# modelscope/KAN-TTS

Measured on AMD Instinct MI355X. Metric: mel-frames/sec (SAM-BERT train), higher is better.
Workload: dtype bf16; 1 GPU; SAM-BERT full (sambert_16k.yaml zhcn) fwd+bwd+clip+Adam, batch 32/GPU, T_in 64, 14797 valid mel frames on rank 0, dropout on; global_batch=32, parallelism=dp1, launch=graph, collective_world_size=1

## Files before the change

include/kantts_hip.h:

```cpp
#ifndef KANTTS_HIP_H
#define KANTTS_HIP_H

#include <stddef.h>
#include <stdint.h>

#ifdef __cplusplus
extern "C" {
#endif

#define KANTTS_OK 0
#define KANTTS_E_BADARG (-1)
#define KANTTS_E_UNSUPPORTED (-2)
#define KANTTS_E_WORKSPACE (-3)

int kantts_abi_version(void);
const char* kantts_target_arch(void);

#define KANTTS_GEMM_MAX_SEG 4
typedef struct kantts_gemm_seg {
  const float* a;
  const float* a_gate;
  const float* b;
  int64_t a_is, a_ks;
  int64_t b_js, b_ks;
// ... 152 lines not shown
                    int64_t* lens, int B, int N, int Tp, void* stream);
int kantts_lr_gather_fwd(const float* x, const int32_t* idx, const int64_t* valid_lens, float* out, int B, int N,
                         int Tp, int C, int ldo, int out_col_offset, void* stream);
int kantts_lr_gather_bwd(const float* dout, const int32_t* cs, const int64_t* valid_lens, float* dx, int B, int N,
                         int Tp, int C, int ldo, int out_col_offset, int accumulate, void* stream);

int kantts_lr_memory_fwd(const float* aug, const float* spk, const float* emo, const int32_t* idx,
                         const int64_t* valid_lens, const float* pos_enc, float* memory, float* lr_text, float* lr_spk,
                         float* lr_emo, int B, int N, int Tp, int r, int d_t, int d_s, int d_e, void* stream);
int kantts_lr_memory_bwd(const float* d_memory, long long ldm, const int32_t* cs, const int64_t* valid_lens, float* d_aug,
                         float* d_spk, float* d_emo, int B, int N, int Tp, int r, int d_t, int d_s, int d_e, void* stream);

int kantts_fsmn_dwconv_fwd(const float* x, const float* w, const float* res, const int64_t* lens, float* y, int B,
                           int T, int C, int K, int left_pad, void* stream);
int kantts_fsmn_dwconv_fwd_rows(const float* x, const float* w, const float* res, const int64_t* lens, float* y, int B,
                                int T, int C, int K, int left_pad, int t0, int t1, void* stream);
int kantts_fsmn_dwconv_fwd_slots(const float* x, const float* w, const float* res, const int64_t* lens, float* y, int B,
                                 int T, int C, int K, int left_pad, const int32_t* t0, const int32_t* t1, int max_rows,
                                 void* stream);
int kantts_fsmn_dwconv_bwd(const float* dy, const float* x, const float* w, const int64_t* lens, float* dx,
                           float* dw_accum, float* workspace, long long ws_floats, int B, int T, int C, int K,
                           int left_pad, void* stream);
long long kantts_fsmn_dwconv_bwd_ws(int B, int T, int C, int K);
int kantts_fsmn_memory_drop_fwd(const float* c, const float* w, const float* res, const int64_t* lens, float* y, int B,
                                int T, int C, int K, int left_pad, float p1, uint64_t seed1, float p2, uint64_t seed2,
                                const uint64_t* seed_dev, void* stream);
int kantts_fsmn_memory_drop_bwd(const float* dy, const float* w, const int64_t* lens, float* dx, float* dym, int B, int T,
                                int C, int K, int left_pad, float p1, uint64_t seed1, float p2, uint64_t seed2,
                                const uint64_t* seed_dev, void* stream);
typedef struct kantts_fsmn_drop_args {
  const float* x;
  const float* w;
  const float* res;
  float* y;
  float* dym;
  float p1, p2;
  uint64_t seed1, seed2;
} kantts_fsmn_drop_args;
int kantts_fsmn_memory_drop_fwd_pair(const kantts_fsmn_drop_args* a, const kantts_fsmn_drop_args* b, const int64_t* lens,
                                     int B, int T, int C, int K, int left_pad, const uint64_t* seed_dev, void* stream);
int kantts_fsmn_memory_drop_bwd_pair(const kantts_fsmn_drop_args* a, const kantts_fsmn_drop_args* b, const int64_t* lens,
                                     int B, int T, int C, int K, int left_pad, const uint64_t* seed_dev, void* stream);

int kantts_masked_l1(const float* pred, const float* target, const int64_t* lens, float* loss_accum, float* grad,
                     int B, int T, int C, void* stream);

// ... 803 lines not shown
```

kan-tts_amd/csrc/seq.hip:

```cpp
#include "common.h"

struct EmbedArgs {
  const float* tab[4];
  int ntab;
  const int64_t* ids;
  const float* pos;
  float* out;
  float* scaled;
  int rows, T, D;
  float scale;
};

__global__ void embed_sum_kernel(const EmbedArgs a) {
  long long idx = (long long)blockIdx.x * blockDim.x + threadIdx.x;
  long long total = (long long)a.rows * a.D;
  if (idx >= total) return;
  int row = (int)(idx / a.D), d = (int)(idx % a.D);
  float s = 0.f;
  for (int k = 0; k < a.ntab; ++k) s += a.tab[k][(long long)a.ids[(long long)row * a.ntab + k] * a.D + d];
  s *= a.scale;
  if (a.scaled) a.scaled[idx] = s;
  if (a.pos) s += a.pos[(long long)(row % a.T) * a.D + d];
  a.out[idx] = s;
}
// ... 448 lines not shown
      const int t = t0 + o;
      const bool ok = t < (ROWS ? min(len, r1) : len);
      const float v = xb[(long long)(ok ? t : 0) * C + c];
      ctr[o] = ok ? v : 0.f;
    }
#pragma unroll
    for (int o = 0; o < FS_TT; ++o) {
      const int t = t0 + o;
      float acc = ctr[o];
#pragma unroll
      for (int k = 0; k < FS_K; ++k) acc = fmaf(wk[k], xin[o + k], acc);
      if (t < tlim) {
        const long long oidx = ((long long)b * T + t) * C + c;
        float outv = (t < len) ? acc : 0.f;
        if (!FLIP && res) outv += res[oidx];
        y[oidx] = outv;
      }
    }
  }
}

#define FS_CH 128
#define FS_SUB (FS_CH / 4)
__global__ __launch_bounds__(256) void fsmn_dw41_partial_kernel(const float* __restrict__ dy, const float* __restrict__ x,
                                                            const int64_t* __restrict__ lens,
                                                            float* __restrict__ part, int B, int T, int C, int lp) {
  __shared__ float sm[4][FS_K][65];
  const int b = blockIdx.y, chunk = blockIdx.x, nchunk = gridDim.x;
  const int wave = threadIdx.x >> 6, lane = threadIdx.x & 63;
  const int c0 = blockIdx.z * 64, c = c0 + lane;
  const bool cok = c < C;
  const int cc = cok ? c : 0;
  const int len = lens ? (int)min((long long)lens[b], (long long)T) : T;
  const float* xb = x + (long long)b * T * C;
  const float* db = dy + (long long)b * T * C;
  const int tbeg = chunk * FS_CH + wave * FS_SUB, tend = min(tbeg + FS_SUB, T);
  float acc[FS_K];
#pragma unroll
  for (int k = 0; k < FS_K; ++k) acc[k] = 0.f;
  for (int t0 = tbeg; t0 < tend && t0 < len; t0 += FS_TT) {
    float xin[FS_TT + FS_K - 1], dv[FS_TT];
#pragma unroll
    for (int n = 0; n < FS_TT + FS_K - 1; ++n) {
      const int ts = t0 + n - lp;
      const bool ok = cok && (ts >= 0) && (ts < len);
      const float v = xb[(long long)(ok ? ts : 0) * C + cc];
      xin[n] = ok ? v : 0.f;
    }
#pragma unroll
    for (int o = 0; o < FS_TT; ++o) {
      const int t = t0 + o;
      const bool ok = cok && (t < tend) && (t < len);
      const float v = db[(long long)(ok ? t : 0) * C + cc];
      dv[o] = ok ? v : 0.f;
    }
    __builtin_amdgcn_sched_barrier(0);
#pragma unroll
    for (int o = 0; o < FS_TT; ++o)
#pragma unroll
      for (int k = 0; k < FS_K; ++k) acc[k] = fmaf(dv[o], xin[o + k], acc[k]);
  }
#pragma unroll
  for (int k = 0; k < FS_K; ++k) sm[wave][k][lane] = acc[k];
  __syncthreads();
  float* p = part + (((long long)b * nchunk + chunk) * C + c0) * FS_K;
  const int nout = min(64, C - c0) * FS_K;
  for (int o = threadIdx.x; o < nout; o += 256) {
    const int cl = o / FS_K, k = o - cl * FS_K;
    p[o] = (sm[0][k][cl] + sm[1][k][cl]) + (sm[2][k][cl] + sm[3][k][cl]);
  }
}

#define FS_RS 8
__global__ __launch_bounds__(64 * FS_RS) void fsmn_dw_reduce_kernel(const float* __restrict__ part, float* __restrict__ dw,
                                                                    int nblk, int n) {
  __shared__ float sm[FS_RS][64];
  const int lane = threadIdx.x & 63, slice = threadIdx.x >> 6;
  const int i = blockIdx.x * 64 + lane;
  const bool ok = i < n;
  const long long ii = ok ? i : 0;
  float s0 = 0.f, s1 = 0.f, s2 = 0.f, s3 = 0.f;
  int p = slice;
  for (; p + 3 * FS_RS < nblk; p += 4 * FS_RS) {
    const float a0 = part[(long long)p * n + ii], a1 = part[(long long)(p + FS_RS) * n + ii];
    const float a2 = part[(long long)(p + 2 * FS_RS) * n + ii], a3 = part[(long long)(p + 3 * FS_RS) * n + ii];
    s0 += a0, s1 += a1, s2 += a2, s3 += a3;
  }
  for (; p < nblk; p += FS_RS) s0 += part[(long long)p * n + ii];
  sm[slice][lane] = (s0 + s1) + (s2 + s3);
  __syncthreads();
  if (slice == 0 && ok) {
    float s = 0.f;
#pragma unroll
    for (int q = 0; q < FS_RS; ++q) s += sm[q][lane];
    dw[i] += s;
  }
}

static int fs_xcd_order() {
  static const bool off = getenv("KANTTS_FIR_NO_XCD_ORDER") != nullptr;
  return off ? 0 : 1;
}

extern "C" long long kantts_fsmn_dwconv_bwd_ws(int B, int T, int C, int K) {
  if (K != FS_K) return 0;
  return (long long)B * kantts_cdiv(T, FS_CH) * C * K;
}

extern "C" int kantts_fsmn_dwconv_fwd(const float* x, const float* w, const float* res, const int64_t* lens, float* y,
                                      int B, int T, int C, int K, int left_pad, void* stream) {
  if (!x || !w || !y || B < 0 || T < 0 || C < 1 || K < 1) return KANTTS_E_BADARG;
  if (B == 0 || T == 0) return KANTTS_OK;
  const int threads = C >= 256 ? 256 : (C >= 128 ? 128 : 64);
  if (K == FS_K) {
    hipLaunchKernelGGL((fsmn_fir41_kernel<false, 0>), dim3(kantts_cdiv(T, FS_TT), B), dim3(threads), 0,
                       (hipStream_t)stream, x, w, res, lens, y, B, T, C, left_pad, fs_xcd_order(), 0, T,
                       (const int32_t*)nullptr, (const int32_t*)nullptr, 0);
  } else {
    hipLaunchKernelGGL(fsmn_dwconv_fwd_kernel<0>, dim3(kantts_cdiv(T, DW_TT), B), dim3(threads), 0, (hipStream_t)stream, x,
// ... 47 lines not shown
    const int nchunk = kantts_cdiv(T, FS_CH);
    if (dw_accum && (!workspace || ws_floats < (long long)B * nchunk * C * K)) return KANTTS_E_WORKSPACE;
    if (dx)
      hipLaunchKernelGGL((fsmn_fir41_kernel<true, 0>), dim3(kantts_cdiv(T, FS_TT), B), dim3(threads), 0, st, dy,
                         w, (const float*)nullptr, lens, dx, B, T, C, left_pad, fs_xcd_order(), 0, T, (const int32_t*)nullptr,
                         (const int32_t*)nullptr, 0);
    if (dw_accum) {
      hipLaunchKernelGGL(fsmn_dw41_partial_kernel, dim3(nchunk, B, kantts_cdiv(C, 64)), dim3(256), 0, st, dy, x, lens,
                         workspace, B, T, C, left_pad);
      hipLaunchKernelGGL(fsmn_dw_reduce_kernel, dim3(kantts_cdiv(C * K, 64)), dim3(64 * FS_RS), 0, st, workspace, dw_accum,
                         B * nchunk, C * K);
    }
  } else {
    if (dx)
      hipLaunchKernelGGL(fsmn_dwconv_bwd_dx_kernel, dim3(kantts_cdiv(T, DW_TT), B), dim3(threads), 0, st, dy, w, lens, dx,
                         B, T, C, K, left_pad);
    if (dw_accum)
      hipLaunchKernelGGL(fsmn_dwconv_bwd_dw_kernel, dim3(kantts_cdiv(T, DW_WT), B), dim3(threads), 0, st, dy, x, lens,
                         dw_accum, B, T, C, K, left_pad);
  }
  KANTTS_CHECK_LAUNCH();
}

__global__ __launch_bounds__(256) void teacher_plan_kernel(const kantts_plan_args g) {
  const long long nA = (long long)g.B * g.N, nB = (long long)g.B * g.T_mel, L = g.Tp / g.r, nC = (long long)g.B * L;
  const long long nD = (long long)g.B * g.Tp * g.depth, nE = (long long)g.B * L * g.d_mel, nF = g.B;
  const long long total = nA + nB + nC + nD + nE + nF;
  for (long long i = (long long)blockIdx.x * blockDim.x + threadIdx.x; i < total; i += (long long)gridDim.x * blockDim.x) {
    long long k = i;
    if (k < nA) {
      const int b = (int)(k / g.N), n = (int)(k % g.N);
      const long long len = min(g.in_lens[b], (long long)g.N);
      g.in_mask[k] = n >= len ? 1 : 0;
      g.prev[k] = logf((n > 0 ? (float)g.dur[k - 1] : 0.f) + 1.f);
      continue;
    }
    k -= nA;
    if (k < nB) {
      const int b = (int)(k / g.T_mel), t = (int)(k % g.T_mel);
      g.out_mask[k] = t >= min(g.out_lens[b], (long long)g.T_mel) ? 1 : 0;
      continue;
    }
    k -= nB;
    if (k < nC) {
      const int b = (int)(k / L), l = (int)(k % L);
      g.lfr_mask[k] = l >= min((g.out_lens[b] + g.r - 1) / g.r, L) ? 1 : 0;
// ... 69 lines not shown
```

kan-tts_amd/kantts/_hip/__init__.py:

```python
import ctypes
import os
from ctypes import (POINTER, Structure, c_char_p, c_float, c_int, c_int32, c_int64, c_longlong,
                    c_uint64, c_void_p)

import torch

_HERE = os.path.dirname(os.path.abspath(__file__))
LIB_PATH = os.environ.get("KANTTS_LIB") or os.path.normpath(os.path.join(_HERE, "..", "..", "libkantts_hip.so"))
_lib = None

GEMM_MAX_SEG = 4
PREC_FP32, PREC_BF16, PREC_REF = 0, 1, 2


class GemmSeg(Structure):
    _fields_ = [
        ("a", c_void_p), ("a_gate", c_void_p), ("b", c_void_p),
        ("a_is", c_int64), ("a_ks", c_int64), ("b_js", c_int64), ("b_ks", c_int64), ("b_tap", c_int64),
        ("klen", c_int32), ("ntaps", c_int32),
        ("a_tok_axis", c_int32), ("a_shift0", c_int32), ("a_shift_step", c_int32),
        ("b_tok_axis", c_int32), ("b_shift0", c_int32), ("b_shift_step", c_int32),
        ("a_drop_p", c_float), ("a_drop_seed", c_uint64),
        ("a_inner", c_int32), ("a_Tq", c_int32), ("a_Tsrc", c_int32), ("a_mul", c_int32), ("a_div", c_int32),
        ("a_up", c_int32),
# ... 329 lines not shown


class EncAttnArgs(Structure):
    _fields_ = [("x", c_void_p), ("xn", c_void_p), ("lens", c_void_p), ("rowmask", c_void_p), ("wqkv", c_void_p),
                ("bqkv", c_void_p), ("wfc", c_void_p), ("bfc", c_void_p), ("ln1_gamma", c_void_p), ("ln1_beta", c_void_p),
                ("ln1_eps", c_float), ("att_p", c_float), ("fc_p", c_float), ("att_seed", c_uint64), ("fc_seed", c_uint64),
                ("seed_dev", c_void_p), ("qkv", c_void_p), ("o", c_void_p), ("lse", c_void_p), ("y1", c_void_p),
                ("xn1", c_void_p), ("xn1_bf16", c_int32), ("mean1", c_void_p), ("rstd1", c_void_p), ("B", c_int32),
                ("L", c_int32)]


class CtcArgs(Structure):
    _fields_ = [("logits", c_void_p), ("in_lens", c_void_p), ("out_lens", c_void_p), ("ws", c_void_p), ("loss", c_void_p),
                ("grad", c_void_p), ("B", c_int32), ("T1", c_int32), ("T2", c_int32), ("blank", c_float),
                ("grad_scale", c_float)]


ROWSUM_MAX = 32


class RowSumArgs(Structure):
    _fields_ = [("n", c_int32), ("cols", c_int32), ("split", c_int32), ("rows", c_int32 * ROWSUM_MAX),
                ("src", c_void_p * ROWSUM_MAX), ("dst0", c_void_p * ROWSUM_MAX), ("dst1", c_void_p * ROWSUM_MAX)]


class FragMajorDesc(Structure):
    _fields_ = [("src_off", c_int64), ("dst_off", c_int64), ("sr", c_int64), ("sk", c_int64), ("R", c_int32),
                ("K", c_int32)]


class TapMajorDesc(Structure):
    _fields_ = [("src_off", c_int64), ("dst_off", c_int64), ("N", c_int32), ("Cin", c_int32), ("KT", c_int32),
                ("pad_", c_int32)]


def available() -> bool:
    return os.path.exists(LIB_PATH)


def lib():
    global _lib
    if _lib is None:
        if not os.path.exists(LIB_PATH):
            raise RuntimeError(
                "libkantts_hip.so is not built (%s). Run `python -c 'import __graft_entry__ as g; g.build()'` "
                "or `make -C kan-tts_amd/csrc`. There is no CPU fallback." % LIB_PATH)
# ... 12 lines not shown
        L.kantts_pnca_attn_bwd.argtypes = [p, p, i, p, p, p, p, p, p, p, p, p, p, p, i, i, i, i, i, i, f, u64, u64, p, p]
        L.kantts_attn_plan.argtypes = [i, i, i]
        L.kantts_lstm_fwd.argtypes = [p, p, p, p, p, p, p, i, i, i, i, i, i, p]
        L.kantts_attn_decode.argtypes = [p, p, p, i, i, i, p, i, p, p, i, i, i, i, i, i, i, p]
        L.kantts_lstm_cell.argtypes = [p, p, p, p, i, i, p]
        L.kantts_mas_width1.argtypes = [p, p, p, p, p, i, i, i, p]
        L.kantts_align_attn_fwd.argtypes = [p, p, p, p, p, p, i, i, i, i, p]
        L.kantts_align_attn_bwd.argtypes = [p, p, p, p, p, p, p, p, p, p, i, i, i, i, p]
        L.kantts_lstm_bwd.argtypes = [p, p, p, p, p, p, i, i, i, i, i, i, p]
        L.kantts_embed_sum_fwd.argtypes = [POINTER(c_void_p), i, p, p, p, p, i, i, i, f, p]
        L.kantts_embed_sum_bwd.argtypes = [POINTER(c_void_p), i, p, p, i, i, f, p]
        L.kantts_lr_index.argtypes = [p, p, p, p, p, p, i, i, i, p]
        L.kantts_lr_gather_fwd.argtypes = [p, p, p, p, i, i, i, i, i, i, p]
        L.kantts_lr_gather_bwd.argtypes = [p, p, p, p, i, i, i, i, i, i, i, p]
        L.kantts_lr_memory_fwd.argtypes = [p, p, p, p, p, p, p, p, p, p, i, i, i, i, i, i, i, p]
        L.kantts_lr_memory_bwd.argtypes = [p, ll, p, p, p, p, p, i, i, i, i, i, i, i, p]
        L.kantts_fsmn_dwconv_fwd.argtypes = [p, p, p, p, p, i, i, i, i, i, p]
        L.kantts_fsmn_dwconv_bwd.argtypes = [p, p, p, p, p, p, p, ll, i, i, i, i, i, p]
        L.kantts_fsmn_dwconv_bwd_ws.argtypes = [i, i, i, i]
        L.kantts_fsmn_dwconv_bwd_ws.restype = ll
        if hasattr(L, "kantts_fsmn_memory_drop_fwd") and hasattr(L, "kantts_fsmn_memory_drop_bwd"):
            L.kantts_fsmn_memory_drop_fwd.argtypes = [p, p, p, p, p, i, i, i, i, i, f, u64, f, u64, p, p]
            L.kantts_fsmn_memory_drop_bwd.argtypes = [p, p, p, p, p, i, i, i, i, i, f, u64, f, u64, p, p]
        L.kantts_masked_l1.argtypes = [p, p, p, p, p, i, i, i, p]
        L.kantts_sumsq.argtypes = [p, p, ll, p]
        L.kantts_elem_loss.argtypes = [p, p, f, i, f, p, p, ll, p]
        L.kantts_adam_step.argtypes = [p, p, p, p, ll, f, f, f, f, f, f, f, p, f, p, p]
        L.kantts_melspec_fwd.argtypes = [p, i, i, i, i, i, i, p, p, f, p, p, p, p, i, f, p, p, p]
        L.kantts_melspec_norm_fwd.argtypes = [p, i, i, i, i, i, i, p, p, f, p, p, p, p, i, f, f, f, f, i, p, p, p]
        L.kantts_melspec_bwd.argtypes = [p, p, i, i, i, i, i, i, p, p, f, p, p, p, p, i, f, p, p]
        L.kantts_melspec_norm_fwd_fm.argtypes = [p, i, i, i, i, i, i, p, p, f, p, p, p, p, i, f, f, f, f, i, i, p, p, p]
        L.kantts_melspec_bwd_fm.argtypes = [p, p, i, i, i, i, i, i, p, p, f, p, p, p, p, i, f, i, p, p]
        L.kantts_weight_norm_fwd.argtypes = [p, p, p, i, i, p]
        L.kantts_weight_norm_bwd.argtypes = [p, p, p, p, p, i, i, p]
        L.kantts_weight_norm_strided_fwd.argtypes = [p, p, p, i, i, i, ll, ll, ll, p]
        L.kantts_weight_norm_strided_bwd.argtypes = [p, p, p, p, p, i, i, i, ll, ll, ll, p]
        L.kantts_sinadd_fwd.argtypes = [p, p, ll, p]
        L.kantts_sinadd_bwd.argtypes = [p, p, p, ll, p]
        L.kantts_conv_win_launch.argtypes = [POINTER(ConvArgs), c_void_p]
        L.kantts_conv_wgrad_launch.argtypes = [POINTER(ConvWArgs), c_void_p]
        L.kantts_conv_c1_launch.argtypes = [POINTER(ConvC1Args), c_int, c_void_p]
        L.kantts_pnca_decode_step.argtypes = [p, i, p, p, p, p, p, p, i, i, i, i, i, p, i, p]
        L.kantts_step_rows.argtypes = [p, p, i, i, ll, ll, ll, ll, i, p, p]
        L.kantts_step_rowmask.argtypes = [p, p, i, i, p, p]
        L.kantts_upsample_stream.argtypes = [p, p, p, p, p, i, i, i, i, i, f, i, p]
        L.kantts_sinadd_lrelu_fwd.argtypes = [p, p, p, f, ll, p]
# ... 129 lines not shown
    "kantts_bgemm_nt", "kantts_ffn_pair", "kantts_fragmajor_bf16", "kantts_bgemm_tn", "kantts_cast_f32_bf16", "kantts_tapmajor_bf16", "kantts_relu_gate_bf16",
    "kantts_ln128_fwd", "kantts_ln128_bwd", "kantts_ln128_bwd_rows", "kantts_bgemm_nt_lnbwd", "kantts_stft_mag_bwd", "kantts_bgemm_tn_grouped", "kantts_sumsq_det",
    "kantts_pnca_decode_step", "kantts_step_rows", "kantts_step_rowmask", "kantts_upsample_stream",
    "kantts_sinadd_lrelu_fwd", "kantts_dropout2_add",
    "kantts_cconv_launch", "kantts_cconv_wgrad_launch", "kantts_cconv_wgrad_ws_floats", "kantts_act_cast_bf16",
    "kantts_ragged_rows_f32", "kantts_ragged_rows_i64", "kantts_weight_norm_tap_images",
    "kantts_weight_norm_table", "kantts_weight_norm_table_bwd", "kantts_masked_l1_many", "kantts_scale_many",
    "kantts_mean_many", "kantts_scale_to_many", "kantts_elem_loss_many", "kantts_conv_n1_launch",
    "kantts_pnca_block_fwd", "kantts_pnca_block_bwd", "kantts_pnca_block_bwd_ws_floats", "kantts_rows_sum_many",
    "kantts_melspec_tuning", "kantts_teacher_plan", "kantts_copy_roof", "kantts_pnca_attn_qkv_bwd",
    "kantts_pnca_decode_run", "kantts_pnca_decode_blob_sizes", "kantts_dur_ar_run", "kantts_dur_ar_run_f32", "kantts_ctc_attn", "kantts_ctc_attn_workspace", "kantts_enc_attn_fwd",
    "kantts_launch_tuning", "kantts_sconv_launch", "kantts_sconv_rows_launch",
    "kantts_pnca_decode_range", "kantts_lstm_fwd_range", "kantts_fsmn_dwconv_fwd_rows",
    "kantts_pnca_decode_slots", "kantts_lstm_fwd_slots", "kantts_fsmn_dwconv_fwd_slots", "kantts_scatter_rows_f32",
    "kantts_nsf_source_rows", "kantts_nsf_downs_rows", "kantts_mel_handover_rows",
    "kantts_mb_tail_rows", "kantts_sconv_sym_rows_launch", "kantts_lr_memory_fwd", "kantts_lr_memory_bwd",
    "kantts_nsf_source_end_rows", "kantts_nsf_downs_sym_rows", "kantts_nsf_draw_states", "kantts_nsf_source_wgrad",
    *FP_SYMBOLS, "kantts_fp_plan_given",
    *SPK_SYMBOLS,
    "kantts_fsmn_memory_drop_fwd", "kantts_fsmn_memory_drop_bwd",
    *PREDICTOR_PAIR_SYMBOLS,
    *CORPUS_PRIOR_SYMBOLS,
    *SYBERT_SYMBOLS,
]


_launch_tuning = [None]


def apply_launch_tuning():
    L = lib()
    env = os.environ
    want = (id(L), int(env.get("KANTTS_TN_TILE", "0") or 0), int(env.get("KANTTS_TN_SLICES", "0") or 0),
            int(env.get("KANTTS_C1_WGRAD_WGS", "0") or 0))
    if want != _launch_tuning[0]:
        rc = L.kantts_launch_tuning(want[1], max(want[2], 0), max(want[3], 0))
        if rc != 0:
            raise RuntimeError("libkantts_hip: launch_tuning failed with code %d" % rc)
        _launch_tuning[0] = want


def check(rc, what):
    if rc != 0:
        raise RuntimeError("libkantts_hip: %s failed with code %d" % (what, rc))


# ... 603 lines not shown
        _profile_families.append(("pnca_attn_qkv_bwd", e0, e1, flops, float(nbytes)))
    return ws


def rows_sum_many(problems):
    for s0 in range(0, len(problems), ROWSUM_MAX):
        chunk = problems[s0:s0 + ROWSUM_MAX]
        g = RowSumArgs()
        g.n, g.cols, g.split = len(chunk), 256, 128
        for i, (src, d0, d1) in enumerate(chunk):
            assert src.dim() == 2 and src.shape[1] == 256 and src.is_contiguous()
            g.rows[i] = int(src.shape[0])
            g.src[i], g.dst0[i], g.dst1[i] = _addr(src), _addr(d0), _addr(d1)
        check(lib().kantts_rows_sum_many(ctypes.byref(g), stream()), "rows_sum_many")


def rows_sum_accum(src, dst0, dst1):
    if deferred_tn.enabled:
        deferred_tn.rowsums.append((src, deferred_tn._desc(dst0), deferred_tn._desc(dst1)))
        return
    rows_sum_many([(src, dst0, dst1)])


TN_MAX_GROUP = 16


class _DeferredTN:

    def __init__(self):
        self.enabled = False
        self.groups = {}
        self.copies = []
        self.rowsums = []

    def add(self, key, g, a, b, c, db, seed, keep):
        self.groups.setdefault(key, []).append((g, a, b, c, db, seed, keep))

    @staticmethod
    def _desc(t):
        return (t.untyped_storage(), t.storage_offset(), tuple(t.shape), tuple(t.stride()), t.dtype, t.device)

    @staticmethod
    def _rebuild(d):
        st, off, shape, stride, dtype, dev = d
        return torch.empty(0, dtype=dtype, device=dev).set_(st, off, shape, stride)

    def shared_gradient(self, src):
        if not self.enabled:
            return src
        from .ops import gzeros

        dst = gzeros(tuple(src.shape), src.device) if src.dtype == torch.float32 else torch.empty_like(src)
        self.copies.append((self._desc(dst), self._desc(src)))
        return dst

    def flush(self):
        if not self.groups and not self.copies and not self.rowsums:
            return
        groups, self.groups = self.groups, {}
        copies, self.copies = self.copies, []
        rowsums, self.rowsums = self.rowsums, []
        self._launch([probs[s:s + TN_MAX_GROUP] for probs in groups.values() for s in range(0, len(probs), TN_MAX_GROUP)])
        if rowsums:
            rows_sum_many([(src, self._rebuild(d0), self._rebuild(d1)) for src, d0, d1 in rowsums])
        if copies:
            torch._foreach_copy_([self._rebuild(d) for d, _ in copies], [self._rebuild(s) for _, s in copies])

    def _launch(self, chunks):
        L = lib()
        for chunk in chunks:
            n = len(chunk)
            arr = lambda k: (c_void_p * n)(*[q[k] for q in chunk])
            seeds = (c_uint64 * n)(*[q[5] for q in chunk])
            g = chunk[0][0]
            g.slices = 0
            if _profile is not None:
                e0, e1 = torch.cuda.Event(enable_timing=True), torch.cuda.Event(enable_timing=True)
                e0.record()
            apply_launch_tuning()
            check(L.kantts_bgemm_tn_grouped(ctypes.byref(g), n, arr(1), arr(2), arr(3), arr(4), seeds, stream()),
                  "bgemm_tn_grouped")
            if _profile is not None:
                e1.record()
                _profile.append((e0, e1, 2.0 * g.M * g.N * g.K * g.ntaps * n))


deferred_tn = _DeferredTN()
# ... 749 lines not shown
```

kan-tts_amd/kantts/_hip/ops.py:

```python
import itertools
import os
import weakref
import math

import torch

from . import (E_UNSUPPORTED, act_cast_bf16, bgemm_nt, bgemm_tn, cconv, cconv_wgrad, check, get_precision, conv_c1, conv_n1, conv_wgrad,
               conv_win, gemm, lib, make_seg, nsf_source, nsf_source_wgrad, ptr, rng_state, stream)
from . import ops_bf16

_seed_counter = itertools.count(1)


def next_seed():
    return (torch.initial_seed() * 0x9E3779B97F4A7C15 + next(_seed_counter) * 0xD1B54A32D192ED03) & ((1 << 63) - 1)


def _c(t):
    return t if t.is_contiguous() else t.contiguous()


def distinct_stream(priority=None):
    taken = {st.cuda_stream for st in helper_streams()} | {torch.cuda.current_stream().cuda_stream}
    for _ in range(64):
# ... 100 lines not shown
                return self
            if o._stream is None:
                o._stream = _new_side_stream()
            ev = torch.cuda.Event()
            ev.record(torch.cuda.current_stream())
            o._stream.wait_event(ev)
            self.cm = torch.cuda.stream(o._stream)
            self.cm.__enter__()
            o._keep.extend(t for t in self.keep if t is not None)
            o._used = True
            return self

        def __exit__(self, *exc):
            if self.cm is not None:
                self.cm.__exit__(*exc)
            return False

    def side(self, *keep):
        return _WgradOverlap._Ctx(self, keep)

    def flush_early(self):
        from . import deferred_tn

        if not self.enabled or not (deferred_tn.groups or deferred_tn.copies or deferred_tn.rowsums):
            return
        keep = [k for probs in deferred_tn.groups.values() for q in probs for k in q[6] if k is not None]
        keep += [r[0] for r in deferred_tn.rowsums]
        with self.side(*keep):
            deferred_tn.flush()

    def join(self):
        from . import deferred_tn

        deferred_tn.flush()
        flush_weight_norm_backward()
        side_branch.join()
        side_branch.release()
        if self._used:
            ev = torch.cuda.Event()
            ev.record(self._stream)
            torch.cuda.current_stream().wait_event(ev)
            self._keep.clear()
            self._used = False


wgrad_overlap = _WgradOverlap()


_branch_streams = []

# ... 1032 lines not shown
def lr_memory_entry_points():
    return hasattr(lib(), "kantts_lr_memory_fwd")


def lr_memory(aug, spk, emo, idx, cs, valid_lens, pos_enc, r, frames=None):
    B, Tp = idx.shape
    if (LR_MEMORY["on"] and Tp % r == 0 and not pos_enc.requires_grad and lr_memory_entry_points()
            and tuple(pos_enc.shape) == (B, Tp, aug.shape[-1])
            and all(t.dtype == torch.float32 for t in (aug, spk, emo, pos_enc))):
        try:
            mem, text, fs, fe = _LRMemory.apply(_c(aug), _c(spk), _c(emo), idx, cs, valid_lens, _c(pos_enc), int(r),
                                                frames is None)
            return (mem, text) + ((fs, fe) if frames is None else tuple(frames))
        except _LRMemoryDeclined:
            pass
    text = lr_gather(aug, idx, cs, valid_lens) + pos_enc
    fs, fe = frames if frames is not None else (lr_gather(spk, idx, cs, valid_lens), lr_gather(emo, idx, cs, valid_lens))
    ds, de = spk.shape[-1], emo.shape[-1]
    mem = torch.cat([text.reshape(B, -1, r * text.shape[-1]), fs.reshape(B, -1, r * ds)[:, :, :ds],
                     fe.reshape(B, -1, r * de)[:, :, :de]], dim=-1)
    return mem, text, fs, fe


class _FsmnMemory(torch.autograd.Function):
    @staticmethod
    def forward(ctx, x, w, res, lens, lp):
        x, w = _c(x), _c(w)
        B, T, C = x.shape
        K = w.shape[-1]
        y = torch.empty_like(x)
        r = _c(res) if res is not None else None
        check(lib().kantts_fsmn_dwconv_fwd(ptr(x, torch.float32), ptr(w, torch.float32), ptr(r), ptr(lens), ptr(y), B,
                                           T, C, K, int(lp), stream()), "fsmn_dwconv_fwd")
        ctx.save_for_backward(x, w, lens)
        ctx.cfg = (B, T, C, K, int(lp), res is not None)
        return y

    @staticmethod
    def backward(ctx, dy):
        x, w, lens = ctx.saved_tensors
        B, T, C, K, lp, has_res = ctx.cfg
        dy = _c(dy)
        dx = torch.empty_like(x)
        dw = gzeros_like(w)
        ws_n = int(lib().kantts_fsmn_dwconv_bwd_ws(B, T, C, K))
        ws = torch.empty(max(ws_n, 1), device=dy.device, dtype=torch.float32)
        check(lib().kantts_fsmn_dwconv_bwd(ptr(dy, torch.float32), ptr(x), ptr(w), ptr(lens), ptr(dx), None, None, 0,
                                           B, T, C, K, lp, stream()), "fsmn_dwconv_bwd (dx)")
        with wgrad_overlap.side(dy, x, ws):
            check(lib().kantts_fsmn_dwconv_bwd(ptr(dy, torch.float32), ptr(x), ptr(w), ptr(lens), None, ptr(dw), ptr(ws),
                                               ws_n, B, T, C, K, lp, stream()), "fsmn_dwconv_bwd (dw)")
        return dx, dw, (dy if has_res else None), None, None


def fsmn_memory(x, w, lens_i64, left_pad, res=None):
    return _FsmnMemory.apply(x, w, res, lens_i64, left_pad)


class _FsmnMemoryDrop(torch.autograd.Function):

    @staticmethod
    def forward(ctx, c, w, res, lens, lp, p1, p2, res_grad=None):
        from . import rng_ptr

        c, w = _c(c), _c(w)
        B, T, C = c.shape
        K = w.shape[-1]
        r = None if res is None else _c(res)
        y = torch.empty_like(c)
        s1 = next_seed() if p1 > 0 else 0
        s2 = next_seed() if p2 > 0 else 0
        rc = lib().kantts_fsmn_memory_drop_fwd(ptr(c, torch.float32), ptr(w, torch.float32), ptr(r, torch.float32),
                                               ptr(lens), ptr(y), B, T, C, K, int(lp), float(p1), s1, float(p2), s2,
                                               rng_ptr(c.device), stream())
# ... 6 lines not shown
        check(rc, "fsmn_memory_drop_fwd")
        ctx.save_for_backward(c, w, lens)
        ctx.cfg = (B, T, C, K, int(lp), float(p1), s1, float(p2), s2, res is not None)
        ctx.res_grad = res_grad if (res is not None and res_grad is not None and res_grad.armed) else None
        return y

    @staticmethod
    def backward(ctx, dy):
        from . import rng_ptr

        c, w, lens = ctx.saved_tensors
        B, T, C, K, lp, p1, s1, p2, s2, has_res = ctx.cfg
        dy = _c(dy)
        dx, dym = torch.empty_like(c), torch.empty_like(c)
        rc = lib().kantts_fsmn_memory_drop_bwd(ptr(dy, torch.float32), ptr(w), ptr(lens), ptr(dx), ptr(dym), B, T, C, K, lp,
                                               p1, s1, p2, s2, rng_ptr(dy.device), stream())
        if rc == E_UNSUPPORTED:
            check(lib().kantts_dropout2_add(ptr(dy), None, ptr(dym), dy.numel(), p1, s1, p2, s2, rng_ptr(dy.device),
                                            stream()), "dropout2_add")
            rc = lib().kantts_fsmn_dwconv_bwd(ptr(dym), ptr(c), ptr(w), ptr(lens), ptr(dx), None, None, 0, B, T, C, K, lp,
                                              stream())
        check(rc, "fsmn_memory_drop_bwd")
        dw = gzeros_like(w)
        ws_n = int(lib().kantts_fsmn_dwconv_bwd_ws(B, T, C, K))
        ws = torch.empty(max(ws_n, 1), device=dy.device, dtype=torch.float32)
        with wgrad_overlap.side(dym, c, ws):
            check(lib().kantts_fsmn_dwconv_bwd(ptr(dym), ptr(c), ptr(w), ptr(lens), None, ptr(dw), ptr(ws), ws_n, B, T, C,
                                               K, lp, stream()), "fsmn_dwconv_bwd (dw)")
        d_res = dy if has_res and ctx.needs_input_grad[2] else None
        if d_res is not None and ctx.res_grad is not None:
            ctx.res_grad.dres, d_res = d_res, None
        return dx, dw, d_res, None, None, None, None, None


FSMN_MEMORY_DROP = {"on": not os.environ.get("KANTTS_NO_FSMN_MEMORY_DROP")}


def fsmn_memory_drop_entry_points():
    L = lib()
    return hasattr(L, "kantts_fsmn_memory_drop_fwd") and hasattr(L, "kantts_fsmn_memory_drop_bwd")


def fsmn_memory_drop(x, w, lens_i64, left_pad, p1=0.0, p2=0.0, res=None, res_grad=None):
    if (FSMN_MEMORY_DROP["on"] and x.dtype == torch.float32 and w.dtype == torch.float32 and w.shape[-1] == 41
            and x.dim() == 3 and x.shape[-1] % 4 == 0 and (res is None or (res.shape == x.shape and res.dtype == x.dtype))
            and fsmn_memory_drop_entry_points()):
        return _FsmnMemoryDrop.apply(x, w, res, lens_i64, left_pad, float(p1), float(p2), res_grad)
    return dropout2_add(fsmn_memory(x, w, lens_i64, left_pad), p1, p2, res, res_grad=res_grad)


def _fsmn_drop_args(x, w, res, y, dym, p1, s1, p2, s2):
# ... 22 lines not shown
        check(lib().kantts_fsmn_memory_drop_fwd_pair(ctypes.byref(a), ctypes.byref(b), ptr(lens), B, T, C, K, int(lp),
                                                     rng_ptr(cs[0].device), stream()), "fsmn_memory_drop_fwd_pair")
        ctx.save_for_backward(lens, *cs, *ws)
        ctx.cfg = (B, T, C, K, int(lp), cfgs, [r is not None for r in rs])
        ctx.res_grads = [tok if (r is not None and tok is not None and tok.armed) else None for r, tok in zip(rs, res_grads)]
        return ys[0], ys[1]

    @staticmethod
    def backward(ctx, dya, dyb):
        import ctypes

        from . import rng_ptr

        lens, ca, cb, wa, wb = ctx.saved_tensors
        B, T, C, K, lp, cfgs, has_res = ctx.cfg
        cs, ws, dys = [ca, cb], [wa, wb], [_c(dya), _c(dyb)]
        dxs, dyms = [torch.empty_like(c) for c in cs], [torch.empty_like(c) for c in cs]
        a, b = (_fsmn_drop_args(dy, w, None, dx, dym, *cfg) for dy, w, dx, dym, cfg in zip(dys, ws, dxs, dyms, cfgs))
        check(lib().kantts_fsmn_memory_drop_bwd_pair(ctypes.byref(a), ctypes.byref(b), ptr(lens), B, T, C, K, lp,
                                                     rng_ptr(dys[0].device), stream()), "fsmn_memory_drop_bwd_pair")
        out = []
        for i, (c, w, dy, dx, dym) in enumerate(zip(cs, ws, dys, dxs, dyms)):
            dw = gzeros_like(w)
            ws_n = int(lib().kantts_fsmn_dwconv_bwd_ws(B, T, C, K))
            wsp = torch.empty(max(ws_n, 1), device=dy.device, dtype=torch.float32)
            with wgrad_overlap.side(dym, c, wsp):
                check(lib().kantts_fsmn_dwconv_bwd(ptr(dym), ptr(c), ptr(w), ptr(lens), None, ptr(dw), ptr(wsp), ws_n, B, T, C,
                                                   K, lp, stream()), "fsmn_dwconv_bwd (dw)")
            d_res = dy if has_res[i] and ctx.needs_input_grad[6 + 3 * i] else None
            if d_res is not None and ctx.res_grads[i] is not None:
                ctx.res_grads[i].dres, d_res = d_res, None
            out += [dx, dw, d_res]
        return (None, None, None, None, *out)


def fsmn_memory_drop2(xs, ws, lens_i64, left_pad, cfgs, ress=(None, None), res_grads=(None, None)):
    return _FsmnMemoryDrop2.apply(lens_i64, int(left_pad), [tuple(c) for c in cfgs], list(res_grads), xs[0], ws[0], ress[0],
                                  xs[1], ws[1], ress[1])


class _MaskedL1(torch.autograd.Function):
    @staticmethod
    def forward(ctx, pred, target, lens):
        pred, target = _c(pred), _c(target)
        if pred.dim() == 2:
            B, T = pred.shape
            C = 1
        else:
            B, T, C = pred.shape
        loss = torch.zeros((), device=pred.device, dtype=torch.float32)
        need_grad = ctx.needs_input_grad[0]
# ... 1554 lines not shown
```

kan-tts_amd/kantts/train/segments.py:

```python
import gc

import torch
import torch.distributed as dist

from kantts._hip import ops


def all_ranks_agree(ok, device):
    if not (dist.is_available() and dist.is_initialized()) or dist.get_world_size() <= 1:
        return bool(ok)
    on_host = dist.get_backend() == "gloo"
    flag = torch.tensor([1 if ok else 0], dtype=torch.int32, device="cpu" if on_host else device)
    dist.all_reduce(flag, op=dist.ReduceOp.MIN)
    return bool(int(flag.item()))


class SegmentedCapture:
    def __init__(self, arenas, stream):
        self.arenas, self.stream = list(arenas), stream
        self.segments = []
        self._graph = self._pool = None
        self.skip_exchange = False

    def _cut(self, arena, bucket):
# ... 26 lines not shown
                out = fn()
                ops.join_capturing_side_streams()
                self._graph.capture_end()
                self.segments.append((self._graph, None, None, False))
                self._graph = None
        finally:
            self._restore_arenas()
        torch.cuda.current_stream().wait_stream(self.stream)
        want = sum(len(a.buckets) for a in self.arenas) + 1
        if len(self.segments) != want:
            raise RuntimeError("expected %d segments, captured %d" % (want, len(self.segments)))
        return out

    def _restore_arenas(self):
        saved = getattr(self, "_saved", None) or [(False, False)] * len(self.arenas)
        for a, (overlap, _) in zip(self.arenas, saved):
            a.bucket_ready = a.capture_stream = None
            a.overlap, a._active = overlap, False
        self._saved = None

    def abort(self):
        from kantts._hip import deferred_tn

        deferred_tn.groups, deferred_tn.copies, deferred_tn.rowsums = {}, [], []
        self._restore_arenas()
        try:
            with torch.cuda.stream(self.stream):
                if self._graph is not None and torch.cuda.is_current_stream_capturing():
                    ops.join_capturing_side_streams()
                    self._graph.capture_end()
        except Exception:
            pass
        self._graph = None
        self.segments = []
        torch.cuda.synchronize()

    def replay(self):
        pending = {}
        for g, arena, bucket, last in self.segments:
            g.replay()
            if arena is None or self.skip_exchange:
                continue
            pending.setdefault(id(arena), []).append(arena.exchange(bucket))
            if last:
                for h in pending.pop(id(arena)):
                    h.wait()
```

Baseline: 3.082 million mel-frames/s.

## Batch FSMN depthwise filter-gradient kernels into deferred grouped launches

Adds a multi-problem kernel pair (partial + reduce) that computes the 41-tap FSMN depthwise weight gradients for up to 16 layers in one launch. The weight-gradient calls are queued in the deferred flush mechanism, with event waits for cross-stream producers, instead of being launched one by one on the wgrad overlap side stream. This is meant to cut per-layer launch overhead and improve GPU fill for small per-layer grids. In exchange, these gradients run later and serialised at flush time rather than overlapped, and tensors must be kept alive until the flush.

```diff
diff --git a/include/kantts_hip.h b/include/kantts_hip.h
--- a/include/kantts_hip.h
+++ b/include/kantts_hip.h
@@ -198,6 +198,17 @@
                            float* dw_accum, float* workspace, long long ws_floats, int B, int T, int C, int K,
                            int left_pad, void* stream);
 long long kantts_fsmn_dwconv_bwd_ws(int B, int T, int C, int K);
+#define KANTTS_FIR_DW_MAX 16
+typedef struct kantts_fir_dw_problem {
+  const float* dy;
+  const float* x;
+  const int64_t* lens;
+  float* dw_accum;
+  float* workspace;
+  long long ws_floats;
+  int32_t B, T, C, left_pad;
+} kantts_fir_dw_problem;
+int kantts_fsmn_dw41_many(const kantts_fir_dw_problem* probs, int nprob, void* stream);
 int kantts_fsmn_memory_drop_fwd(const float* c, const float* w, const float* res, const int64_t* lens, float* y, int B,
                                 int T, int C, int K, int left_pad, float p1, uint64_t seed1, float p2, uint64_t seed2,
                                 const uint64_t* seed_dev, void* stream);
diff --git a/kan-tts_amd/csrc/seq.hip b/kan-tts_amd/csrc/seq.hip
--- a/kan-tts_amd/csrc/seq.hip
+++ b/kan-tts_amd/csrc/seq.hip
@@ -1,3 +1,5 @@
+#include <limits.h>
+
 #include "common.h"
 
 struct EmbedArgs {
@@ -494,13 +496,12 @@
 
 #define FS_CH 128
 #define FS_SUB (FS_CH / 4)
-__global__ __launch_bounds__(256) void fsmn_dw41_partial_kernel(const float* __restrict__ dy, const float* __restrict__ x,
-                                                            const int64_t* __restrict__ lens,
-                                                            float* __restrict__ part, int B, int T, int C, int lp) {
-  __shared__ float sm[4][FS_K][65];
-  const int b = blockIdx.y, chunk = blockIdx.x, nchunk = gridDim.x;
+__device__ __forceinline__ void fsmn_dw41_partial_body(const float* __restrict__ dy, const float* __restrict__ x,
+                                                       const int64_t* __restrict__ lens, float* __restrict__ part, int T,
+                                                       int C, int lp, int chunk, int nchunk, int b, int cgroup,
+                                                       float (*sm)[FS_K][65]) {
   const int wave = threadIdx.x >> 6, lane = threadIdx.x & 63;
-  const int c0 = blockIdx.z * 64, c = c0 + lane;
+  const int c0 = cgroup * 64, c = c0 + lane;
   const bool cok = c < C;
   const int cc = cok ? c : 0;
   const int len = lens ? (int)min((long long)lens[b], (long long)T) : T;
@@ -543,12 +544,40 @@
   }
 }
 
+__global__ __launch_bounds__(256) void fsmn_dw41_partial_kernel(const float* __restrict__ dy, const float* __restrict__ x,
+                                                            const int64_t* __restrict__ lens,
+                                                            float* __restrict__ part, int B, int T, int C, int lp) {
+  __shared__ float sm[4][FS_K][65];
+  fsmn_dw41_partial_body(dy, x, lens, part, T, C, lp, blockIdx.x, gridDim.x, blockIdx.y, blockIdx.z, sm);
+}
+
+struct FirDwManyArgs {
+  const float* dy[KANTTS_FIR_DW_MAX];
+  const float* x[KANTTS_FIR_DW_MAX];
+  const int64_t* lens[KANTTS_FIR_DW_MAX];
+  float* part[KANTTS_FIR_DW_MAX];
+  float* dw[KANTTS_FIR_DW_MAX];
+  int B[KANTTS_FIR_DW_MAX], T[KANTTS_FIR_DW_MAX], C[KANTTS_FIR_DW_MAX], lp[KANTTS_FIR_DW_MAX];
+  int pend[KANTTS_FIR_DW_MAX], rend[KANTTS_FIR_DW_MAX];
+  int nprob;
+};
+
+__global__ __launch_bounds__(256) void fsmn_dw41_partial_many_kernel(const FirDwManyArgs g) {
+  __shared__ float sm[4][FS_K][65];
+  const int id = blockIdx.x;
+  int q = 0;
+  while (q < g.nprob - 1 && id >= g.pend[q]) ++q;
+  const int local = id - (q ? g.pend[q - 1] : 0);
+  const int T = g.T[q], B = g.B[q], nchunk = (T + FS_CH - 1) / FS_CH;
+  const int chunk = local % nchunk, rest = local / nchunk;
+  fsmn_dw41_partial_body(g.dy[q], g.x[q], g.lens[q], g.part[q], T, g.C[q], g.lp[q], chunk, nchunk, rest % B, rest / B, sm);
+}
+
 #define FS_RS 8
-__global__ __launch_bounds__(64 * FS_RS) void fsmn_dw_reduce_kernel(const float* __restrict__ part, float* __restrict__ dw,
-                                                                    int nblk, int n) {
-  __shared__ float sm[FS_RS][64];
+__device__ __forceinline__ void fsmn_dw_reduce_body(const float* __restrict__ part, float* __restrict__ dw, int nblk, int n,
+                                                    int blk, float (*sm)[64]) {
   const int lane = threadIdx.x & 63, slice = threadIdx.x >> 6;
-  const int i = blockIdx.x * 64 + lane;
+  const int i = blk * 64 + lane;
   const bool ok = i < n;
   const long long ii = ok ? i : 0;
   float s0 = 0.f, s1 = 0.f, s2 = 0.f, s3 = 0.f;
@@ -567,6 +596,21 @@
     for (int q = 0; q < FS_RS; ++q) s += sm[q][lane];
     dw[i] += s;
   }
+}
+
+__global__ __launch_bounds__(64 * FS_RS) void fsmn_dw_reduce_kernel(const float* __restrict__ part, float* __restrict__ dw,
+                                                                    int nblk, int n) {
+  __shared__ float sm[FS_RS][64];
+  fsmn_dw_reduce_body(part, dw, nblk, n, blockIdx.x, sm);
+}
+
+__global__ __launch_bounds__(64 * FS_RS) void fsmn_dw_reduce_many_kernel(const FirDwManyArgs g) {
+  __shared__ float sm[FS_RS][64];
+  const int id = blockIdx.x;
+  int q = 0;
+  while (q < g.nprob - 1 && id >= g.rend[q]) ++q;
+  const int nblk = g.B[q] * ((g.T[q] + FS_CH - 1) / FS_CH);
+  fsmn_dw_reduce_body(g.part[q], g.dw[q], nblk, g.C[q] * FS_K, id - (q ? g.rend[q - 1] : 0), sm);
 }
 
 static int fs_xcd_order() {
@@ -660,6 +704,31 @@
   KANTTS_CHECK_LAUNCH();
 }
 
+extern "C" int kantts_fsmn_dw41_many(const kantts_fir_dw_problem* probs, int nprob, void* stream) {
+  if (nprob < 0 || nprob > KANTTS_FIR_DW_MAX || (nprob > 0 && !probs)) return KANTTS_E_BADARG;
+  FirDwManyArgs g = {};
+  long long pend = 0, rend = 0;
+  for (int i = 0; i < nprob; ++i) {
+    const kantts_fir_dw_problem& p = probs[i];
+    if (!p.dy || !p.x || !p.dw_accum || p.B < 0 || p.T < 0 || p.C < 1 || p.C > INT_MAX / FS_K) return KANTTS_E_BADARG;
+    if (p.B == 0 || p.T == 0) continue;
+    const long long nchunk = kantts_cdiv(p.T, FS_CH);
+    if (!p.workspace || p.ws_floats < (long long)p.B * nchunk * p.C * FS_K) return KANTTS_E_WORKSPACE;
+    pend += nchunk * p.B * kantts_cdiv(p.C, 64);
+    rend += kantts_cdiv(p.C * FS_K, 64);
+    if (pend > INT_MAX || (long long)p.B * nchunk > INT_MAX) return KANTTS_E_UNSUPPORTED;
+    const int n = g.nprob++;
+    g.dy[n] = p.dy, g.x[n] = p.x, g.lens[n] = p.lens, g.part[n] = p.workspace, g.dw[n] = p.dw_accum;
+    g.B[n] = p.B, g.T[n] = p.T, g.C[n] = p.C, g.lp[n] = p.left_pad;
+    g.pend[n] = (int)pend, g.rend[n] = (int)rend;
+  }
+  if (g.nprob == 0) return KANTTS_OK;
+  hipStream_t st = (hipStream_t)stream;
+  hipLaunchKernelGGL(fsmn_dw41_partial_many_kernel, dim3((unsigned)pend), dim3(256), 0, st, g);
+  hipLaunchKernelGGL(fsmn_dw_reduce_many_kernel, dim3((unsigned)rend), dim3(64 * FS_RS), 0, st, g);
+  KANTTS_CHECK_LAUNCH();
+}
+
 __global__ __launch_bounds__(256) void teacher_plan_kernel(const kantts_plan_args g) {
   const long long nA = (long long)g.B * g.N, nB = (long long)g.B * g.T_mel, L = g.Tp / g.r, nC = (long long)g.B * L;
   const long long nD = (long long)g.B * g.Tp * g.depth, nE = (long long)g.B * L * g.d_mel, nF = g.B;
diff --git a/kan-tts_amd/kantts/_hip/__init__.py b/kan-tts_amd/kantts/_hip/__init__.py
--- a/kan-tts_amd/kantts/_hip/__init__.py
+++ b/kan-tts_amd/kantts/_hip/__init__.py
@@ -375,6 +375,14 @@
 class RowSumArgs(Structure):
     _fields_ = [("n", c_int32), ("cols", c_int32), ("split", c_int32), ("rows", c_int32 * ROWSUM_MAX),
                 ("src", c_void_p * ROWSUM_MAX), ("dst0", c_void_p * ROWSUM_MAX), ("dst1", c_void_p * ROWSUM_MAX)]
+
+
+FIR_DW_MAX = 16
+
+
+class FirDwProblem(Structure):
+    _fields_ = [("dy", c_void_p), ("x", c_void_p), ("lens", c_void_p), ("dw_accum", c_void_p), ("workspace", c_void_p),
+                ("ws_floats", c_longlong), ("B", c_int32), ("T", c_int32), ("C", c_int32), ("left_pad", c_int32)]
 
 
 class FragMajorDesc(Structure):
@@ -433,6 +441,8 @@
         if hasattr(L, "kantts_fsmn_memory_drop_fwd") and hasattr(L, "kantts_fsmn_memory_drop_bwd"):
             L.kantts_fsmn_memory_drop_fwd.argtypes = [p, p, p, p, p, i, i, i, i, i, f, u64, f, u64, p, p]
             L.kantts_fsmn_memory_drop_bwd.argtypes = [p, p, p, p, p, i, i, i, i, i, f, u64, f, u64, p, p]
+        if hasattr(L, "kantts_fsmn_dw41_many"):
+            L.kantts_fsmn_dw41_many.argtypes = [POINTER(FirDwProblem), i, p]
         L.kantts_masked_l1.argtypes = [p, p, p, p, p, i, i, i, p]
         L.kantts_sumsq.argtypes = [p, p, ll, p]
         L.kantts_elem_loss.argtypes = [p, p, f, i, f, p, p, ll, p]
@@ -608,6 +618,7 @@
     *PREDICTOR_PAIR_SYMBOLS,
     *CORPUS_PRIOR_SYMBOLS,
     *SYBERT_SYMBOLS,
+    "kantts_fsmn_dw41_many",
 ]
 
 
@@ -1257,6 +1268,36 @@
     rows_sum_many([(src, dst0, dst1)])
 
 
+def fir_dw_many_entry_point():
+    return hasattr(lib(), "kantts_fsmn_dw41_many")
+
+
+def fir_dw_many(problems):
+    s0 = 0
+    while s0 < len(problems):
+        chunk, seen = [], set()
+        for q in problems[s0:s0 + FIR_DW_MAX]:
+            if ptr(q[3]) in seen:
+                break
+            seen.add(ptr(q[3]))
+            chunk.append(q)
+        s0 += len(chunk)
+        arr = (FirDwProblem * len(chunk))()
+        for g, (dy, x, lens, dw, ws, ws_n, B, T, C, lp) in zip(arr, chunk):
+            g.dy, g.x, g.lens = ptr(dy, torch.float32), ptr(x, torch.float32), ptr(lens, torch.int64)
+            g.dw_accum, g.workspace, g.ws_floats = ptr(dw, torch.float32), ptr(ws, torch.float32), int(ws_n)
+            g.B, g.T, g.C, g.left_pad = int(B), int(T), int(C), int(lp)
+        check(lib().kantts_fsmn_dw41_many(arr, len(chunk), stream()), "fsmn_dw41_many")
+
+
+def fir_dw_accum(dy, x, lens, dw, ws, ws_n, B, T, C, lp):
+    ev = sid = None
+    if dy.is_cuda:
+        ev, sid = torch.cuda.Event(), torch.cuda.current_stream().cuda_stream
+        ev.record()
+    deferred_tn.firs.append((dy, x, lens, deferred_tn._desc(dw), ws, ws_n, B, T, C, lp, sid, ev))
+
+
 TN_MAX_GROUP = 16
 
 
@@ -1267,6 +1308,16 @@
         self.groups = {}
         self.copies = []
         self.rowsums = []
+        self.firs = []
+
+    def pending(self):
+        return bool(self.groups or self.copies or self.rowsums or self.firs)
+
+    def discard(self):
+        self.groups, self.copies, self.rowsums, self.firs = {}, [], [], []
+
+    def fir_keep(self):
+        return [t for q in self.firs for t in (q[0], q[1], q[4])]
 
     def add(self, key, g, a, b, c, db, seed, keep):
         self.groups.setdefault(key, []).append((g, a, b, c, db, seed, keep))
@@ -1290,14 +1341,23 @@
         return dst
 
     def flush(self):
-        if not self.groups and not self.copies and not self.rowsums:
+        if not self.pending():
             return
         groups, self.groups = self.groups, {}
         copies, self.copies = self.copies, []
         rowsums, self.rowsums = self.rowsums, []
+        firs, self.firs = self.firs, []
         self._launch([probs[s:s + TN_MAX_GROUP] for probs in groups.values() for s in range(0, len(probs), TN_MAX_GROUP)])
         if rowsums:
             rows_sum_many([(src, self._rebuild(d0), self._rebuild(d1)) for src, d0, d1 in rowsums])
+        if firs:
+            here, last = torch.cuda.current_stream() if firs[0][0].is_cuda else None, {}
+            for q in firs:
+                if q[11] is not None and q[10] != here.cuda_stream:
+                    last[q[10]] = q[11]
+            for ev in last.values():
+                here.wait_event(ev)
+            fir_dw_many([q[:3] + (self._rebuild(q[3]),) + q[4:10] for q in firs])
         if copies:
             torch._foreach_copy_([self._rebuild(d) for d, _ in copies], [self._rebuild(s) for _, s in copies])
 
diff --git a/kan-tts_amd/kantts/_hip/ops.py b/kan-tts_amd/kantts/_hip/ops.py
--- a/kan-tts_amd/kantts/_hip/ops.py
+++ b/kan-tts_amd/kantts/_hip/ops.py
@@ -146,10 +146,11 @@
     def flush_early(self):
         from . import deferred_tn
 
-        if not self.enabled or not (deferred_tn.groups or deferred_tn.copies or deferred_tn.rowsums):
+        if not self.enabled or not deferred_tn.pending():
             return
         keep = [k for probs in deferred_tn.groups.values() for q in probs for k in q[6] if k is not None]
         keep += [r[0] for r in deferred_tn.rowsums]
+        keep += deferred_tn.fir_keep()
         with self.side(*keep):
             deferred_tn.flush()
 
@@ -1228,6 +1229,19 @@
     return mem, text, fs, fe
 
 
+def _fsmn_filter_grad(dy, x, w, lens, dw, B, T, C, K, lp):
+    from . import deferred_tn, fir_dw_accum, fir_dw_many_entry_point
+
+    ws_n = int(lib().kantts_fsmn_dwconv_bwd_ws(B, T, C, K))
+    ws = torch.empty(max(ws_n, 1), device=dy.device, dtype=torch.float32)
+    if deferred_tn.enabled and K == 41 and fir_dw_many_entry_point():
+        fir_dw_accum(dy, x, lens, dw, ws, ws_n, B, T, C, lp)
+        return
+    with wgrad_overlap.side(dy, x, ws):
+        check(lib().kantts_fsmn_dwconv_bwd(ptr(dy, torch.float32), ptr(x), ptr(w), ptr(lens), None, ptr(dw), ptr(ws), ws_n,
+                                           B, T, C, K, lp, stream()), "fsmn_dwconv_bwd (dw)")
+
+
 class _FsmnMemory(torch.autograd.Function):
     @staticmethod
     def forward(ctx, x, w, res, lens, lp):
@@ -1249,13 +1263,9 @@
         dy = _c(dy)
         dx = torch.empty_like(x)
         dw = gzeros_like(w)
-        ws_n = int(lib().kantts_fsmn_dwconv_bwd_ws(B, T, C, K))
-        ws = torch.empty(max(ws_n, 1), device=dy.device, dtype=torch.float32)
         check(lib().kantts_fsmn_dwconv_bwd(ptr(dy, torch.float32), ptr(x), ptr(w), ptr(lens), ptr(dx), None, None, 0,
                                            B, T, C, K, lp, stream()), "fsmn_dwconv_bwd (dx)")
-        with wgrad_overlap.side(dy, x, ws):
-            check(lib().kantts_fsmn_dwconv_bwd(ptr(dy, torch.float32), ptr(x), ptr(w), ptr(lens), None, ptr(dw), ptr(ws),
-                                               ws_n, B, T, C, K, lp, stream()), "fsmn_dwconv_bwd (dw)")
+        _fsmn_filter_grad(dy, x, w, lens, dw, B, T, C, K, lp)
         return dx, dw, (dy if has_res else None), None, None
 
 
@@ -1308,11 +1318,7 @@
                                               stream())
         check(rc, "fsmn_memory_drop_bwd")
         dw = gzeros_like(w)
-        ws_n = int(lib().kantts_fsmn_dwconv_bwd_ws(B, T, C, K))
-        ws = torch.empty(max(ws_n, 1), device=dy.device, dtype=torch.float32)
-        with wgrad_overlap.side(dym, c, ws):
-            check(lib().kantts_fsmn_dwconv_bwd(ptr(dym), ptr(c), ptr(w), ptr(lens), None, ptr(dw), ptr(ws), ws_n, B, T, C,
-                                               K, lp, stream()), "fsmn_dwconv_bwd (dw)")
+        _fsmn_filter_grad(dym, c, w, lens, dw, B, T, C, K, lp)
         d_res = dy if has_res and ctx.needs_input_grad[2] else None
         if d_res is not None and ctx.res_grad is not None:
             ctx.res_grad.dres, d_res = d_res, None
@@ -1381,11 +1387,7 @@
         out = []
         for i, (c, w, dy, dx, dym) in enumerate(zip(cs, ws, dys, dxs, dyms)):
             dw = gzeros_like(w)
-            ws_n = int(lib().kantts_fsmn_dwconv_bwd_ws(B, T, C, K))
-            wsp = torch.empty(max(ws_n, 1), device=dy.device, dtype=torch.float32)
-            with wgrad_overlap.side(dym, c, wsp):
-                check(lib().kantts_fsmn_dwconv_bwd(ptr(dym), ptr(c), ptr(w), ptr(lens), None, ptr(dw), ptr(wsp), ws_n, B, T, C,
-                                                   K, lp, stream()), "fsmn_dwconv_bwd (dw)")
+            _fsmn_filter_grad(dym, c, w, lens, dw, B, T, C, K, lp)
             d_res = dy if has_res[i] and ctx.needs_input_grad[6 + 3 * i] else None
             if d_res is not None and ctx.res_grads[i] is not None:
                 ctx.res_grads[i].dres, d_res = d_res, None
diff --git a/kan-tts_amd/kantts/train/segments.py b/kan-tts_amd/kantts/train/segments.py
--- a/kan-tts_amd/kantts/train/segments.py
+++ b/kan-tts_amd/kantts/train/segments.py
@@ -72,7 +72,7 @@
     def abort(self):
         from kantts._hip import deferred_tn
 
-        deferred_tn.groups, deferred_tn.copies, deferred_tn.rowsums = {}, [], []
+        deferred_tn.discard()
         self._restore_arenas()
         try:
             with torch.cuda.stream(self.stream):
```

Measured after the change: 3.192 million mel-frames/s, median of 6. 3.6% higher.
